# ArrowLuo/SegCLIP

Hardware: AMD Instinct MI355X
Metric: image-text pairs/s fwd+bwd, ViT-B/16 224^2, per-GPU batch 256 (global 2048 at 8 GPUs) (higher is better)
Workload: dtype bf16; 1 GPU; BASELINE configs[1]/[2]: ViT-B/16 224^2 + 77-token text, contrastive loss only; per_gpu_batch=256, global_batch=256, parallelism=dp1, attention_forward=bf16, residual_stream=fp32, cross_mode=t18, text_positions=all 77 (full context, as the reference computes it)

## Files before the change

### segclip_amd/csrc/gemm_bf16_dma.hip

```cpp
#include <stdlib.h>

#include "gemm_bf16_common.h"

namespace {

constexpr int BK = 64;

typedef __attribute__((address_space(3))) void lds_void;
typedef __attribute__((address_space(1))) const void gbl_void;
typedef __attribute__((address_space(3))) s16x4 lds_s16x4;

__device__ __forceinline__ void dma16(const bf16_t* src, char* lds_wave_base) {
  __builtin_amdgcn_global_load_lds((gbl_void*)src, (lds_void*)lds_wave_base, 16, 0, 0);
}

template <int ROWS, int NWV>
__device__ __forceinline__ void issue_direct(const bf16_t* __restrict__ X, int64_t ld, int64_t row0, int64_t nrows,
                                             int64_t k0, char* lds, int wave, int lane) {
  constexpr int PER_WAVE = ROWS / (8 * NWV);
#pragma unroll
  for (int i = 0; i < PER_WAVE; ++i) {
    const int idx = wave * PER_WAVE + i;
    const int row = idx * 8 + (lane >> 3);
    const int chunk = (lane & 7) ^ ((row >> 1) & 7);
    int64_t r = row0 + row;
    r = r < nrows ? r : nrows - 1;
    dma16(X + r * ld + k0 + chunk * 8, lds + idx * 1024);
  }
}
template <int ROWS, int NWV>
__device__ __forceinline__ void issue_ks(const bf16_t* __restrict__ X, int64_t ld, int64_t row0, int64_t nrows,
                                         int64_t k0, char* lds, int wave, int lane) {
  constexpr int PER_WAVE = ROWS / (8 * NWV);
  constexpr int CHUNKS = ROWS / 8;
#pragma unroll
  for (int i = 0; i < PER_WAVE; ++i) {
    const int idx = wave * PER_WAVE + i;
    const int krow = idx * (512 / ROWS) + lane / CHUNKS;
    const int chunk = (lane % CHUNKS) ^ ((krow & 3) << 2);
    int64_t r = row0 + chunk * 8;
    r = r + 8 <= nrows ? r : nrows - 8;
    dma16(X + (k0 + krow) * ld + r, lds + idx * 1024);
  }
}

__device__ __forceinline__ bf16x8_t frag_direct(const char* lds, int rbase, int kc, int lane) {
  const int r = rbase + (lane & 31);
  const int c = kc * 2 + (lane >> 5);
  return *reinterpret_cast<const bf16x8_t*>(lds + r * 128 + ((c ^ ((r >> 1) & 7)) << 4));
}
template <int ROWS>
__device__ __forceinline__ bf16x8_t frag_ks(const char* lds, int rbase, int kc, int lane) {
  const int g4 = lane >> 4, q = lane & 15;
  const int krow = kc * 16 + 8 * (g4 >> 1) + (q >> 2);
  const int col = rbase + 16 * (g4 & 1) + 4 * (q & 3);
  const char* p = lds + krow * (ROWS * 2) + ((((col >> 3) ^ ((krow & 3) << 2))) << 4) + ((col & 7) << 1);
  const s16x4 lo = __builtin_amdgcn_ds_read_tr16_b64_v4i16((lds_s16x4*)(p));
  const s16x4 hi = __builtin_amdgcn_ds_read_tr16_b64_v4i16((lds_s16x4*)(p + 4 * (ROWS * 2)));
  s16x8 r;
  r[0] = lo[0]; r[1] = lo[1]; r[2] = lo[2]; r[3] = lo[3];
  r[4] = hi[0]; r[5] = hi[1]; r[6] = hi[2]; r[7] = hi[3];
  return __builtin_bit_cast(bf16x8_t, r);
}

template <bool A_KS, bool B_KS, int BM, int BN, int NWV>
__global__ __launch_bounds__(NWV * 64, NWV == 4 ? 2 : 1) void gemm_bf16_dma_kernel(Args g) {
  constexpr int SZA = BM * BK * 2;
  constexpr int SZB = BN * BK * 2;
  constexpr int SZS = SZA + SZB;
  constexpr int WN = BN / 64;
  constexpr int WM = NWV / WN;
  constexpr int TM = BM / (WM * 32);
  constexpr int WROWS = TM * 32;
  static_assert(TM == 2 || TM == 4, "wave tile must be 64x64 or 128x64");
  constexpr int LDS_BYTES = 2 * SZS > NWV * EPI_WAVE_BYTES ? 2 * SZS : NWV * EPI_WAVE_BYTES;
  __shared__ __attribute__((aligned(16))) char smem[LDS_BYTES];
  const int tid = threadIdx.x, lane = tid & 63;
  const int wave = __builtin_amdgcn_readfirstlane(tid >> 6);
  const int wm = wave / WN;
  const int wn = wave % WN;
  const int nwg = gridDim.x, bid = blockIdx.x;
  const int q8 = nwg >> 3, r8 = nwg & 7, xcd = bid & 7;
  const int wg = (xcd < r8 ? xcd * (q8 + 1) : r8 * (q8 + 1) + (xcd - r8) * q8) + (bid >> 3);
  const int64_t n0 = (int64_t)(wg % g.nbx) * BN, m0 = (int64_t)(wg / g.nbx) * BM;
  const int64_t z = blockIdx.z, z1 = z / g.nb2, z2 = z % g.nb2;
  const bf16_t* A = reinterpret_cast<const bf16_t*>(g.A) + z1 * g.bsA1 + z2 * g.bsA2;
  const bf16_t* B = g.B + z1 * g.bsB1 + z2 * g.bsB2;
  const int64_t coff = z1 * g.bsC1 + z2 * g.bsC2;
  const int64_t roff = z1 * g.bsR1 + z2 * g.bsR2;

  f32x16 acc[TM][2];
#pragma unroll
  for (int i = 0; i < TM; ++i)
#pragma unroll
    for (int j = 0; j < 2; ++j)
#pragma unroll
      for (int r = 0; r < 16; ++r) acc[i][j][r] = 0.f;

  const int64_t kbeg = (int64_t)blockIdx.y * g.kper;
  const int64_t kend = kbeg + g.kper < g.K ? kbeg + g.kper : g.K;
  const int nk = (int)((kend - kbeg) / BK);

  auto issue = [&](int t) {
    char* la = smem + (t % 2) * SZS;
    char* lb = la + SZA;
    const int64_t k0 = kbeg + (int64_t)t * BK;
    if constexpr (A_KS) issue_ks<BM, NWV>(A, g.lda, m0, g.M, k0, la, wave, lane);
    else issue_direct<BM, NWV>(A, g.lda, m0, g.M, k0, la, wave, lane);
    if constexpr (B_KS) issue_ks<BN, NWV>(B, g.ldb, n0, g.N, k0, lb, wave, lane);
    else issue_direct<BN, NWV>(B, g.ldb, n0, g.N, k0, lb, wave, lane);
  };

  if (NWV == 8 && bid < 256 && gridDim.x * gridDim.y * gridDim.z > 256) {
    const long long t_tile = (long long)nk * 4000 + 20000;
    const long long unit = t_tile / 8 < 5000 ? t_tile / 8 : 5000;
    const long long wait = ((bid >> 3) & 7) * unit;
    const long long t0 = clock64();
    while (clock64() - t0 < wait) __builtin_amdgcn_s_sleep(32);
  }
  issue(0);
  for (int t = 0; t < nk; ++t) {
    asm volatile("s_waitcnt vmcnt(0)" ::: "memory");
    __builtin_amdgcn_s_barrier();
    __builtin_amdgcn_sched_barrier(0);
    if (t + 1 < nk) issue(t + 1);
    const char* la = smem + (t % 2) * SZS;
    const char* lb = la + SZA;
    bf16x8_t fa[2][TM], fb[2][2];
    auto ldfrag = [&](int kc, bf16x8_t (&a)[TM], bf16x8_t (&b)[2]) {
#pragma unroll
      for (int i = 0; i < TM; ++i)
        a[i] = A_KS ? frag_ks<BM>(la, wm * WROWS + i * 32, kc, lane) : frag_direct(la, wm * WROWS + i * 32, kc, lane);
#pragma unroll
      for (int j = 0; j < 2; ++j)
        b[j] = B_KS ? frag_ks<BN>(lb, wn * 64 + j * 32, kc, lane) : frag_direct(lb, wn * 64 + j * 32, kc, lane);
    };
    ldfrag(0, fa[0], fb[0]);
#pragma unroll
    for (int kc = 0; kc < 4; ++kc) {
#pragma unroll
      for (int i = 0; i < TM; ++i) asm volatile("" ::"v"(__builtin_bit_cast(u32x4, fa[kc & 1][i])));
#pragma unroll
      for (int j = 0; j < 2; ++j) asm volatile("" ::"v"(__builtin_bit_cast(u32x4, fb[kc & 1][j])));
      if (kc < 3) ldfrag(kc + 1, fa[(kc + 1) & 1], fb[(kc + 1) & 1]);
      __builtin_amdgcn_sched_barrier(0);
#pragma unroll
      for (int i = 0; i < TM; ++i)
#pragma unroll
        for (int j = 0; j < 2; ++j)
          acc[i][j] = __builtin_amdgcn_mfma_f32_32x32x16_bf16(fa[kc & 1][i], fb[kc & 1][j], acc[i][j], 0, 0, 0);
      __builtin_amdgcn_sched_barrier(0);
    }
  }

  const int64_t mw = m0 + wm * WROWS;
  const int64_t nw = n0 + wn * 64;
  if (g.splits > 1) {
    const int li = lane & 31, lk = lane >> 5;
    float* slab = g.slab + ((int64_t)blockIdx.y * gridDim.z + z) * g.M * g.N;
#pragma unroll
    for (int i = 0; i < TM; ++i)
#pragma unroll
      for (int j = 0; j < 2; ++j) {
        const int64_t n = nw + j * 32 + li;
        if (n >= g.N) continue;
#pragma unroll
        for (int r = 0; r < 16; ++r) {
          const int64_t m = mw + i * 32 + (r & 3) + 8 * (r >> 2) + 4 * lk;
          if (m < g.M) __builtin_nontemporal_store(acc[i][j][r], &slab[m * g.N + n]);
        }
      }
    return;
  }
  const bool full = m0 + BM <= g.M && n0 + BN <= g.N;
#ifdef SEGCLIP_NO_EPILOGUE
  if (acc[0][0][0] != 12345.678f) return;
#endif
  const bool vec = full && g.vec_epi;
  if (vec) __syncthreads();
  float* t = reinterpret_cast<float*>(smem + wave * EPI_WAVE_BYTES);
#define RUN_EPI(SUB, MROW)                                                                              \
  do {                                                                                                  \
    if (vec) {                                                                                          \
      if (g.c_dtype == SEGCLIP_BF16) epilogue_lds_mode<bf16_t>(g, SUB, t, MROW, nw, lane, coff, roff);  \
      else epilogue_lds_mode<float>(g, SUB, t, MROW, nw, lane, coff, roff);                             \
    } else {                                                                                            \
      if (g.c_dtype == SEGCLIP_BF16) epilogue_mode<bf16_t, false>(g, SUB, MROW, nw, 0, 0, lane, coff, roff); \
      else epilogue_mode<float, false>(g, SUB, MROW, nw, 0, 0, lane, coff, roff);                       \
    }                                                                                                   \
  } while (0)
  if constexpr (TM == 2) {
    RUN_EPI(acc, mw);
  } else {
    f32x16 lo[2][2] = {{acc[0][0], acc[0][1]}, {acc[1][0], acc[1][1]}};
    RUN_EPI(lo, mw);
    __builtin_amdgcn_wave_barrier();
    f32x16 hi[2][2] = {{acc[2][0], acc[2][1]}, {acc[3][0], acc[3][1]}};
    RUN_EPI(hi, mw + 64);
  }
#undef RUN_EPI
}

}

#ifndef DMA_PART
#error "compile with -DDMA_PART=0..4 (see build.sh)"
#endif
#define DMA_LAUNCHER(NAME, AK, BKS)                                                                             \
  void NAME(int variant, dim3 grid, hipStream_t stream, const void* args) {                                     \
    const Args g = *reinterpret_cast<const Args*>(args);                                                        \
    if (variant == 2) hipLaunchKernelGGL((gemm_bf16_dma_kernel<AK, BKS, 128, 128, 4>), grid, dim3(256), 0, stream, g); \
    else if (variant == 1) hipLaunchKernelGGL((gemm_bf16_dma_kernel<AK, BKS, 256, 256, 8>), grid, dim3(512), 0, stream, g); \
    else hipLaunchKernelGGL((gemm_bf16_dma_kernel<AK, BKS, 256, 128, 8>), grid, dim3(512), 0, stream, g);       \
  }
#if DMA_PART == 0
DMA_LAUNCHER(segclip_dma_launch_ff, false, false)
#elif DMA_PART == 1
DMA_LAUNCHER(segclip_dma_launch_fk, false, true)
#elif DMA_PART == 2
DMA_LAUNCHER(segclip_dma_launch_kf, true, false)
#elif DMA_PART == 3
DMA_LAUNCHER(segclip_dma_launch_kk, true, true)
#endif

#if DMA_PART == 4
void segclip_dma_launch_ff(int, dim3, hipStream_t, const void*);
void segclip_dma_launch_fk(int, dim3, hipStream_t, const void*);
void segclip_dma_launch_kf(int, dim3, hipStream_t, const void*);
void segclip_dma_launch_kk(int, dim3, hipStream_t, const void*);

static int pick_bn(const segclip_gemm_desc* d, int64_t nbatch_splits) {
  constexpr int BM = 256;
  if (d->N <= 128) return 128;
  auto eff = [&](int bn) {
    const double tiles = (double)cdiv(d->M, BM) * cdiv(d->N, bn) * nbatch_splits;
    const double rounds = tiles / 256.0;
    const double q = rounds / (double)(int64_t)(rounds + 0.999999);
    const double pad = (double)d->N / (cdiv(d->N, bn) * bn);
    return q * pad * (bn == 256 ? 1.0 : 0.72);
  };
  return eff(256) >= eff(128) ? 256 : 128;
}

int segclip_gemm_bf16_dma_pick_bn(const segclip_gemm_desc* d, int64_t nbatch_splits) { return pick_bn(d, nbatch_splits); }

bool segclip_gemm_bf16_dma_try(const segclip_gemm_desc* d, const void* args_, int splits, int64_t kper, int64_t nb,
                               hipStream_t stream) {
  Args g = *reinterpret_cast<const Args*>(args_);
  const bool a_ks = d->sak != 1, b_ks = d->sbk != 1;
  if (d->a_dtype != SEGCLIP_BF16 || d->b_dtype != SEGCLIP_BF16) return false;
  if (d->K % BK != 0 || kper % BK != 0 || d->K < BK) return false;
  if (a_ks && (d->M % 8 != 0 || d->M < 8)) return false;
  if (b_ks && (d->N % 8 != 0 || d->N < 8)) return false;
  if (d->M < 64 || d->N < 16) return false;
  static const int small_rule = segclip_tuning_int("SEGCLIP_GEMM_SMALL_TILES", 1);
  const int bn_big = pick_bn(d, nb * splits);
  const bool colsum_rows128 = g.colsum_part && d->M % 256 != 0;
  const bool small = colsum_rows128 ||
                     (small_rule && d->M >= 128 && d->N >= 128 && !(d->aux_kind == 2 && d->aux) && !g.colsum_part &&
                      cdiv(d->M, 256) * cdiv(d->N, bn_big) * nb * splits < 256);
  const int bn = small ? 128 : bn_big;
  const int bm = small ? 128 : 256;
  g.nbx = (int)cdiv(d->N, bn);
  g.nby = (int)cdiv(d->M, bm);
  g.splits = splits;
  g.kper = kper;
  if (g.colsum_part && bn != 256 && d->N % 128 != 0) return false;
  {
    auto al = [](const void* p) { return p == nullptr || (reinterpret_cast<uintptr_t>(p) & 15) == 0; };
    const int64_t ce = d->c_dtype == SEGCLIP_BF16 ? 8 : 4, re = d->r_dtype == SEGCLIP_BF16 ? 8 : 4;
    g.vec_epi = al(d->C) && al(d->aux) && al(d->residual) && al(d->bias) && d->ldc % ce == 0 &&
                (!d->aux || d->ldaux % ce == 0) && (!d->residual || d->ldr % re == 0) && d->bsC1 % ce == 0 &&
                d->bsC2 % ce == 0 && (!d->residual || (d->bsR1 % re == 0 && d->bsR2 % re == 0));
    if (d->residual && d->r_dtype != d->c_dtype) g.vec_epi = 0;
    if (g.colsum_part && !g.vec_epi) return false;
    if (d->aux_kind == 2 && d->aux && !d->mul_dact && d->act != SEGCLIP_ACT_QUICK_GELU) return false;
    if (d->aux_kind == 2 && d->aux &&
        !(g.vec_epi && d->M % 256 == 0 && d->N % 256 == 0 && d->ldaux % 8 == 0 && d->c_dtype == SEGCLIP_BF16 && splits == 1))
      return false;
  }
  dim3 grid((unsigned)(g.nbx * g.nby), (unsigned)splits, (unsigned)nb);
  const int variant = small ? 2 : bn == 256 ? 1 : 0;
  segclip_gemm_route_note(SEGCLIP_GEMM_ROUTE_DMA, a_ks, b_ks, bm, bn, splits, variant);
  if (!a_ks && !b_ks) segclip_dma_launch_ff(variant, grid, stream, &g);
  else if (!a_ks && b_ks) segclip_dma_launch_fk(variant, grid, stream, &g);
  else if (a_ks && b_ks) segclip_dma_launch_kk(variant, grid, stream, &g);
  else segclip_dma_launch_kf(variant, grid, stream, &g);
  return true;
}
#endif
```

Measured before the change: 7239 pairs/s.

## Add deeper multi-stage LDS DMA pipeline for small-grid bf16 GEMMs

Generalizes the double-buffered direct-to-LDS GEMM into a 2–4 stage operand ring with partial vmcnt waits, so several K tiles of global loads stay in flight. The deeper kernels issue the LDS DMA through inline asm that saves and restores m0 explicitly. A host heuristic enables the deep variants for the 128x128 and 256x128 tiles when the grid fits within about one wave of CUs, with an env override. The aim is to hide memory latency on under-occupied launches, at the cost of more LDS, lower occupancy for the 4-wave kernel, and fragile hand-written m0 handling.

```diff
diff --git a/segclip_amd/csrc/gemm_bf16_dma.hip b/segclip_amd/csrc/gemm_bf16_dma.hip
--- a/segclip_amd/csrc/gemm_bf16_dma.hip
+++ b/segclip_amd/csrc/gemm_bf16_dma.hip
@@ -10,11 +10,20 @@
 typedef __attribute__((address_space(1))) const void gbl_void;
 typedef __attribute__((address_space(3))) s16x4 lds_s16x4;
 
+template <bool HIDDEN>
 __device__ __forceinline__ void dma16(const bf16_t* src, char* lds_wave_base) {
-  __builtin_amdgcn_global_load_lds((gbl_void*)src, (lds_void*)lds_wave_base, 16, 0, 0);
-}
-
-template <int ROWS, int NWV>
+  if constexpr (HIDDEN) {
+    uint32_t keep;
+    asm volatile("s_mov_b32 %0, m0\n\ts_mov_b32 m0, %2\n\ts_nop 0\n\tglobal_load_lds_dwordx4 %1, off\n\ts_mov_b32 m0, %0"
+                 : "=&s"(keep)
+                 : "v"(src), "s"((uint32_t)(uintptr_t)((lds_void*)lds_wave_base))
+                 : "memory");
+  } else {
+    __builtin_amdgcn_global_load_lds((gbl_void*)src, (lds_void*)lds_wave_base, 16, 0, 0);
+  }
+}
+
+template <int ROWS, int NWV, bool HIDDEN>
 __device__ __forceinline__ void issue_direct(const bf16_t* __restrict__ X, int64_t ld, int64_t row0, int64_t nrows,
                                              int64_t k0, char* lds, int wave, int lane) {
   constexpr int PER_WAVE = ROWS / (8 * NWV);
@@ -25,10 +34,10 @@
     const int chunk = (lane & 7) ^ ((row >> 1) & 7);
     int64_t r = row0 + row;
     r = r < nrows ? r : nrows - 1;
-    dma16(X + r * ld + k0 + chunk * 8, lds + idx * 1024);
-  }
-}
-template <int ROWS, int NWV>
+    dma16<HIDDEN>(X + r * ld + k0 + chunk * 8, lds + idx * 1024);
+  }
+}
+template <int ROWS, int NWV, bool HIDDEN>
 __device__ __forceinline__ void issue_ks(const bf16_t* __restrict__ X, int64_t ld, int64_t row0, int64_t nrows,
                                          int64_t k0, char* lds, int wave, int lane) {
   constexpr int PER_WAVE = ROWS / (8 * NWV);
@@ -40,7 +49,7 @@
     const int chunk = (lane % CHUNKS) ^ ((krow & 3) << 2);
     int64_t r = row0 + chunk * 8;
     r = r + 8 <= nrows ? r : nrows - 8;
-    dma16(X + (k0 + krow) * ld + r, lds + idx * 1024);
+    dma16<HIDDEN>(X + (k0 + krow) * ld + r, lds + idx * 1024);
   }
 }
 
@@ -63,8 +72,16 @@
   return __builtin_bit_cast(bf16x8_t, r);
 }
 
-template <bool A_KS, bool B_KS, int BM, int BN, int NWV>
-__global__ __launch_bounds__(NWV * 64, NWV == 4 ? 2 : 1) void gemm_bf16_dma_kernel(Args g) {
+template <int N> __device__ __forceinline__ void wait_vm() {
+  if constexpr (N == 0) asm volatile("s_waitcnt vmcnt(0)" ::: "memory");
+  else if constexpr (N == 6) asm volatile("s_waitcnt vmcnt(6)" ::: "memory");
+  else if constexpr (N == 8) asm volatile("s_waitcnt vmcnt(8)" ::: "memory");
+  else if constexpr (N == 16) asm volatile("s_waitcnt vmcnt(16)" ::: "memory");
+  else static_assert(N < 0, "unsupported vmcnt");
+}
+
+template <bool A_KS, bool B_KS, int BM, int BN, int NWV, int STAGES = 2>
+__global__ __launch_bounds__(NWV * 64, NWV == 4 && STAGES == 2 ? 2 : 1) void gemm_bf16_dma_kernel(Args g) {
   constexpr int SZA = BM * BK * 2;
   constexpr int SZB = BN * BK * 2;
   constexpr int SZS = SZA + SZB;
@@ -73,7 +90,9 @@
   constexpr int TM = BM / (WM * 32);
   constexpr int WROWS = TM * 32;
   static_assert(TM == 2 || TM == 4, "wave tile must be 64x64 or 128x64");
-  constexpr int LDS_BYTES = 2 * SZS > NWV * EPI_WAVE_BYTES ? 2 * SZS : NWV * EPI_WAVE_BYTES;
+  static_assert(STAGES >= 2 && STAGES <= 4, "operand ring of 2..4 stages");
+  constexpr int LDS_BYTES = STAGES * SZS > NWV * EPI_WAVE_BYTES ? STAGES * SZS : NWV * EPI_WAVE_BYTES;
+  constexpr int DMA_PER_STAGE = (BM + BN) / (8 * NWV);
   __shared__ __attribute__((aligned(16))) char smem[LDS_BYTES];
   const int tid = threadIdx.x, lane = tid & 63;
   const int wave = __builtin_amdgcn_readfirstlane(tid >> 6);
@@ -101,14 +120,15 @@
   const int64_t kend = kbeg + g.kper < g.K ? kbeg + g.kper : g.K;
   const int nk = (int)((kend - kbeg) / BK);
 
-  auto issue = [&](int t) {
-    char* la = smem + (t % 2) * SZS;
+  auto issue = [&](int t, int slot) {
+    char* la = smem + slot * SZS;
     char* lb = la + SZA;
     const int64_t k0 = kbeg + (int64_t)t * BK;
-    if constexpr (A_KS) issue_ks<BM, NWV>(A, g.lda, m0, g.M, k0, la, wave, lane);
-    else issue_direct<BM, NWV>(A, g.lda, m0, g.M, k0, la, wave, lane);
-    if constexpr (B_KS) issue_ks<BN, NWV>(B, g.ldb, n0, g.N, k0, lb, wave, lane);
-    else issue_direct<BN, NWV>(B, g.ldb, n0, g.N, k0, lb, wave, lane);
+    constexpr bool HIDDEN = STAGES > 2;
+    if constexpr (A_KS) issue_ks<BM, NWV, HIDDEN>(A, g.lda, m0, g.M, k0, la, wave, lane);
+    else issue_direct<BM, NWV, HIDDEN>(A, g.lda, m0, g.M, k0, la, wave, lane);
+    if constexpr (B_KS) issue_ks<BN, NWV, HIDDEN>(B, g.ldb, n0, g.N, k0, lb, wave, lane);
+    else issue_direct<BN, NWV, HIDDEN>(B, g.ldb, n0, g.N, k0, lb, wave, lane);
   };
 
   if (NWV == 8 && bid < 256 && gridDim.x * gridDim.y * gridDim.z > 256) {
@@ -118,14 +138,27 @@
     const long long t0 = clock64();
     while (clock64() - t0 < wait) __builtin_amdgcn_s_sleep(32);
   }
-  issue(0);
+#pragma unroll
+  for (int p = 0; p < STAGES - 1; ++p)
+    if (p < nk) issue(p, p);
+  int slot = 0;
+  int free_slot = STAGES - 1;
   for (int t = 0; t < nk; ++t) {
-    asm volatile("s_waitcnt vmcnt(0)" ::: "memory");
+    if constexpr (STAGES == 2) {
+      wait_vm<0>();
+    } else {
+      const int after = nk - 1 - t;
+      if (after >= STAGES - 2) wait_vm<(STAGES - 2) * DMA_PER_STAGE>();
+      else if (STAGES == 4 && after == 1) wait_vm<DMA_PER_STAGE>();
+      else wait_vm<0>();
+    }
     __builtin_amdgcn_s_barrier();
     __builtin_amdgcn_sched_barrier(0);
-    if (t + 1 < nk) issue(t + 1);
-    const char* la = smem + (t % 2) * SZS;
+    if (t + STAGES - 1 < nk) issue(t + STAGES - 1, free_slot);
+    const char* la = smem + slot * SZS;
     const char* lb = la + SZA;
+    free_slot = slot;
+    slot = slot + 1 == STAGES ? 0 : slot + 1;
     bf16x8_t fa[2][TM], fb[2][2];
     auto ldfrag = [&](int kc, bf16x8_t (&a)[TM], bf16x8_t (&b)[2]) {
 #pragma unroll
@@ -207,9 +240,11 @@
 #error "compile with -DDMA_PART=0..4 (see build.sh)"
 #endif
 #define DMA_LAUNCHER(NAME, AK, BKS)                                                                             \
-  void NAME(int variant, dim3 grid, hipStream_t stream, const void* args) {                                     \
+  void NAME(int variant, bool deep, dim3 grid, hipStream_t stream, const void* args) {                          \
     const Args g = *reinterpret_cast<const Args*>(args);                                                        \
-    if (variant == 2) hipLaunchKernelGGL((gemm_bf16_dma_kernel<AK, BKS, 128, 128, 4>), grid, dim3(256), 0, stream, g); \
+    if (variant == 2 && deep) hipLaunchKernelGGL((gemm_bf16_dma_kernel<AK, BKS, 128, 128, 4, 4>), grid, dim3(256), 0, stream, g); \
+    else if (variant == 0 && deep) hipLaunchKernelGGL((gemm_bf16_dma_kernel<AK, BKS, 256, 128, 8, 3>), grid, dim3(512), 0, stream, g); \
+    else if (variant == 2) hipLaunchKernelGGL((gemm_bf16_dma_kernel<AK, BKS, 128, 128, 4>), grid, dim3(256), 0, stream, g); \
     else if (variant == 1) hipLaunchKernelGGL((gemm_bf16_dma_kernel<AK, BKS, 256, 256, 8>), grid, dim3(512), 0, stream, g); \
     else hipLaunchKernelGGL((gemm_bf16_dma_kernel<AK, BKS, 256, 128, 8>), grid, dim3(512), 0, stream, g);       \
   }
@@ -224,10 +259,10 @@
 #endif
 
 #if DMA_PART == 4
-void segclip_dma_launch_ff(int, dim3, hipStream_t, const void*);
-void segclip_dma_launch_fk(int, dim3, hipStream_t, const void*);
-void segclip_dma_launch_kf(int, dim3, hipStream_t, const void*);
-void segclip_dma_launch_kk(int, dim3, hipStream_t, const void*);
+void segclip_dma_launch_ff(int, bool, dim3, hipStream_t, const void*);
+void segclip_dma_launch_fk(int, bool, dim3, hipStream_t, const void*);
+void segclip_dma_launch_kf(int, bool, dim3, hipStream_t, const void*);
+void segclip_dma_launch_kk(int, bool, dim3, hipStream_t, const void*);
 
 static int pick_bn(const segclip_gemm_desc* d, int64_t nbatch_splits) {
   constexpr int BM = 256;
@@ -281,11 +316,19 @@
   }
   dim3 grid((unsigned)(g.nbx * g.nby), (unsigned)splits, (unsigned)nb);
   const int variant = small ? 2 : bn == 256 ? 1 : 0;
+  static const int stages_env = segclip_tuning_int("SEGCLIP_GEMM_DMA_STAGES", 0);
+  bool deep = false;
+  if (variant != 1 && stages_env != 2 && kper / BK >= 3) {
+    int dev = 0, ncu = 0;
+    if (!segclip_current_device(&dev, &ncu)) ncu = 256;
+    const int64_t nwg = (int64_t)grid.x * grid.y * grid.z;
+    deep = nwg <= (stages_env == 3 ? 2 * (int64_t)ncu : ncu) || (stages_env == 4 && variant == 2);
+  }
   segclip_gemm_route_note(SEGCLIP_GEMM_ROUTE_DMA, a_ks, b_ks, bm, bn, splits, variant);
-  if (!a_ks && !b_ks) segclip_dma_launch_ff(variant, grid, stream, &g);
-  else if (!a_ks && b_ks) segclip_dma_launch_fk(variant, grid, stream, &g);
-  else if (a_ks && b_ks) segclip_dma_launch_kk(variant, grid, stream, &g);
-  else segclip_dma_launch_kf(variant, grid, stream, &g);
+  if (!a_ks && !b_ks) segclip_dma_launch_ff(variant, deep, grid, stream, &g);
+  else if (!a_ks && b_ks) segclip_dma_launch_fk(variant, deep, grid, stream, &g);
+  else if (a_ks && b_ks) segclip_dma_launch_kk(variant, deep, grid, stream, &g);
+  else segclip_dma_launch_kf(variant, deep, grid, stream, &g);
   return true;
 }
 #endif
```

Result: no change. 7275 pairs/s (median of 6 runs) (+0.5%).
